# janelia-flyem/transfer_em

Hardware: AMD Instinct MI355X
Metric: CycleGAN train steps/sec on 132^3 x1 uint8 volumes (per-GPU batch of 1 volume; aggregate over GPUs) (higher is better)
Workload: dtype f32

## Files before the change

transfer_em_amd/csrc/wino.hip:

```cpp
#include "tem_common.h"
#include "wino_common.h"
#include <cmath>
#include <cstdio>
#include <cstdlib>

namespace wino {

#ifdef TEM_DEBUG_KNOBS
#define KDBG(x) (x)
#else
#define KDBG(x) 0
#endif


struct Ep32 {
  float slope;
  const float *gate; int32_t gN, gD, gH, gW; float gate_slope;
  const uint8_t *keep_mask;
  int32_t doz, doy, dox, dD, dH, dW;
  int32_t gbytes, mbytes;
};

struct Dev {
  const float *in0, *in1;
  int32_t i0N, i0D, i0H, i0W, i1N, i1D, i1H, i1W;
  int32_t C0;
  int32_t N, D, H, W;
  const float *u;
  float *out0, *out1;
  int32_t o0N, o0D, o0H, o0W, o1N, o1D, o1H, o1W;
  int32_t CO0;
  int32_t OD, OH, OW;
  int32_t P;
  int32_t BY, BX, nby, nbx, zsegs, zper, NTZ;
  int32_t E, PLC, subb, slotb;
  int32_t ndma;
  int32_t span0, span1;
  uint32_t magicBX, magicE;
  int32_t dbg;
  int32_t obytes;
  unsigned long long *stamps;
  Ep32 ep;
};

template <int CI, int CO, int NI, int EP, int EE>
__global__ __launch_bounds__(512) void wino_conv_k(Dev p) {
  constexpr int NH = CI / 8, VB = 32;
  constexpr int NB = (CO + 15) / 16;
  constexpr bool STREAM = CI == 32;
  constexpr bool PAIR = CI == 8 && CO == 8;
  constexpr int NKZ = PAIR ? 4 : 3;
  constexpr int UCH = 2 * NB * 16 * 128;
  extern __shared__ __attribute__((aligned(16))) float lds[];
  char *const ring = reinterpret_cast<char *>(lds);
  const int tid = threadIdx.x, lane = tid & 63;
  const int wave = __builtin_amdgcn_readfirstlane(tid >> 6);
  const int m = lane & 15, q = lane >> 4;
  const int grp = PAIR ? wave : (NB == 1 ? wave >> 1 : wave >> 2);
  const int nb = NB == 1 ? 0 : (wave >> 1) & 1;
  const int zb = PAIR ? (q >> 1) : (wave & 1);
  const int co = PAIR ? 4 * (q & 1) : nb * 16 + 4 * q;
  float *const uld = reinterpret_cast<float *>(ring + 4 * p.slotb);

  int seg = (int)xcd_contiguous_block(blockIdx.x, gridDim.x);
  const int zseg = seg % p.zsegs; seg /= p.zsegs;
  const int bx = seg % p.nbx; seg /= p.nbx;
  const int by = seg % p.nby;
  const int n = seg / p.nby;
  const int tz0 = zseg * p.zper, tz1 = min(p.NTZ, tz0 + p.zper), nsteps = tz1 - tz0;
  const int oy0 = by * 2 * p.BY, ox0 = bx * 2 * p.BX;
  const int ntile = p.BY * p.BX;

  const bool two_in = p.in1 != p.in0;
  const float *const in0n = p.in0 + (size_t)n * p.i0N, *const in1n = p.in1 + (size_t)n * p.i1N;
  int voff0[NI], voff1[NI];
  {
    const int iy0 = oy0 - p.P, ix0 = ox0 - p.P;
#pragma unroll
    for (int i = 0; i < NI; ++i) {
      const int sp = (wave + 8 * i) * 64 + lane;
      const bool ex = sp < p.PLC;
      const int spc = ex ? sp : 0;
      const int cpos = spc & 1, ve = spc >> 1;
      const int ro = ve / EE, e = ve - ro * EE;
      const int o = ro & 1, yr = ro >> 1;
      const int c = (cpos ^ swz(e, yr)) * 4;
      const int iy = iy0 + yr, ix = ix0 + 2 * e + o;
      const bool ok = ex && (unsigned)iy < (unsigned)p.H && (unsigned)ix < (unsigned)p.W;
      voff0[i] = ok ? (iy * p.i0H + ix * p.i0W + c) * 4 : (int)0x80000000;
      voff1[i] = ok ? (iy * p.i1H + ix * p.i1W + c) * 4 : (int)0x80000000;
      asm volatile("" : "+v"(voff0[i]), "+v"(voff1[i]));
    }
  }
  auto dma_plane = [&](int iz, int slot) {
    const bool zok = (unsigned)iz < (unsigned)p.D;
    const int izc = zok ? iz : 0;
#pragma unroll
    for (int h = 0; h < NH; ++h) {
      char *const dst = ring + slot * p.slotb + h * p.subb;
      if (!two_in || 8 * h < p.C0)
        dma_subimage<NI, !STREAM>(in0n + izc * p.i0D + 8 * h, zok ? p.span0 - 32 * h : 0, voff0, dst, wave, p.ndma);
      else
        dma_subimage<NI, !STREAM>(in1n + izc * p.i1D + (8 * h - p.C0), zok ? p.span1 - 4 * (8 * h - p.C0) : 0, voff1, dst, wave, p.ndma);
    }
  };

  const int izb0 = 2 * tz0 - p.P;
  if (nsteps > 0) {
#pragma unroll
    for (int k = 0; k < 4; ++k) dma_plane(izb0 + k, k);
  }
  auto dma_u = [&](int chunk, int buf) {
    const __amdgpu_buffer_rsrc_t r = __builtin_amdgcn_make_buffer_rsrc((void *)(p.u + (size_t)chunk * UCH), 0, UCH * 4, 0x00020000);
#pragma unroll
    for (int i = 0; i < UCH * 4 / 1024 / 8; ++i) {
      const int j = wave + 8 * i;
      __builtin_amdgcn_raw_ptr_buffer_load_lds(r, (__attribute__((address_space(3))) void *)((char *)uld + buf * (UCH * 4) + j * 1024), 16,
                                               (j * 64 + lane) * 16, 0, 0, 0);
    }
  };
  if (STREAM) {
    dma_u(0, 0);
  } else {
    constexpr int UF4 = NKZ * NH * NB * 16 * 64 * 2 / 4;
    static_assert(UF4 % 512 == 0, "whole 1 KB wave transfers");
    const __amdgpu_buffer_rsrc_t ur = __builtin_amdgcn_make_buffer_rsrc((void *)p.u, 0, UF4 * 16, 0x00020000);
#pragma unroll
    for (int i = 0; i < UF4 / 512; ++i) {
      const int j = wave + 8 * i;
      __builtin_amdgcn_raw_ptr_buffer_load_lds(ur, (__attribute__((address_space(3))) void *)((char *)uld + j * 1024), 16,
                                               (j * 64 + lane) * 16, 0, 0, 0);
    }
  }
  asm volatile("s_waitcnt vmcnt(0)" ::: "memory");
  __syncthreads();

  constexpr int rowb = EE * VB;
  const Ep32 &ep = p.ep;
  float *const out0n = p.out0 + (size_t)n * p.o0N, *const out1n = EP == 2 ? p.out1 + (size_t)n * p.o1N : nullptr;
  const float *const gaten = EP >= 1 ? ep.gate + (size_t)n * ep.gN : nullptr;
  const bool in0c = EP != 2 || co < p.CO0;
  float *const obase = EP == 2 ? (in0c ? out0n : out1n) : out0n;
  const int oco = in0c ? co : co - p.CO0;
  const int oD = in0c ? p.o0D : p.o1D, oH = in0c ? p.o0H : p.o1H, oW = in0c ? p.o0W : p.o1W;
  const __amdgpu_buffer_rsrc_t grs = __builtin_amdgcn_make_buffer_rsrc((void *)gaten, 0, EP >= 1 ? ep.gbytes : 0, 0x00020000);
  const __amdgpu_buffer_rsrc_t mrs = __builtin_amdgcn_make_buffer_rsrc((void *)ep.keep_mask, 0, EP == 2 ? ep.mbytes : 0, 0x00020000);
  const int mpv = EP == 2 ? p.CO0 >> 3 : 0;
  const int kshift = co & 4;
  int gso[4], mso[4], oso[4];
#pragma unroll
  for (int o4 = 0; o4 < 4; ++o4) {
    gso[o4] = EP >= 1 ? ((o4 >> 1) * ep.gH + (o4 & 1) * ep.gW) * 4 : 0;
    mso[o4] = EP == 2 ? ((o4 >> 1) * ep.dW + (o4 & 1)) * mpv : 0;
    oso[o4] = ((o4 >> 1) * p.o0H + (o4 & 1) * p.o0W) * 4;
  }
  const __amdgpu_buffer_rsrc_t ors = __builtin_amdgcn_make_buffer_rsrc((void *)out0n, 0, EP != 2 ? p.obytes : 0, 0x00020000);

  const int tA = min(grp * 16 + m, ntile - 1);
  const int tyA = (int)fdiv((uint32_t)tA, (uint32_t)p.BX, p.magicBX), txA = tA - tyA * p.BX;
  const int a0 = (4 * tyA * EE + txA) * VB + (q & 1) * 8;
  int cs[2][2];
#pragma unroll
  for (int a = 0; a < 2; ++a)
#pragma unroll
    for (int b = 0; b < 2; ++b) cs[a][b] = ((q >> 1) ^ swz(txA + a, 2 * (tyA + b))) * 16;

#ifdef TEM_DEBUG_KNOBS
  unsigned long long t_last = p.stamps ? clock64() : 0, t_sum[8] = {0, 0, 0, 0, 0, 0, 0, 0};
#define STAMP(i) do { if (p.stamps) { unsigned long long t_now = clock64(); t_sum[i] += t_now - t_last; t_last = t_now; } } while (0)
#else
#define STAMP(i) do { } while (0)
#endif
  f32x4 acc[16];
  f32x4 gv[4];
  uint32_t kb[4];
  uint32_t tyx, tok4 = 0;
  {
    const int t = grp * 16 + m;
    const int ty = (int)fdiv((uint32_t)t, (uint32_t)p.BX, p.magicBX), tx = t - ty * p.BX;
    const int oy = oy0 + 2 * ty, ox = ox0 + 2 * tx;
    const bool tok = co < CO && t < ntile;
#pragma unroll
    for (int o4 = 0; o4 < 4; ++o4) tok4 |= ((tok && oy + (o4 >> 1) < p.OH && ox + (o4 & 1) < p.OW) ? 1u : 0u) << o4;
    tyx = ((uint32_t)oy << 16) | (uint32_t)ox;
  }
  auto tile_geom = [&](int oz, int &o0, int &go, int &mb, uint32_t &okm) {
    uint32_t yx = tyx;
    asm volatile("" : "+v"(yx));
    const int oy = (int)(yx >> 16), ox = (int)(yx & 0xffffu);
    okm = oz < p.OD ? tok4 : 0u;
    o0 = oz * oD + oy * oH + ox * oW + oco;
    go = EP >= 1 ? (oz * ep.gD + oy * ep.gH + ox * ep.gW + co) * 4 : 0;
    mb = EP == 2 ? (int)(((((uint32_t)n * ep.dD + (oz + ep.doz)) * ep.dH + (oy + ep.doy)) * ep.dW + (ox + ep.dox)) * (uint32_t)mpv) + (co >> 3) : 0;
  };
  auto fetch_ep = [&](int oz) {
    int o0, go, mb;
    uint32_t okm;
    tile_geom(oz, o0, go, mb, okm);
    if (!in0c) okm = 0;
#pragma unroll
    for (int o4 = 0; o4 < 4; ++o4) {
      const bool okf = (okm >> o4) & 1u;
      int goff = okf ? go : (int)0x80000000;
      asm volatile("" : "+v"(goff));
      const u32x4 g4 = __builtin_amdgcn_raw_buffer_load_b128(grs, goff, gso[o4], 0);
      gv[o4] = f32x4{__uint_as_float(g4.x), __uint_as_float(g4.y), __uint_as_float(g4.z), __uint_as_float(g4.w)};
      if (EP == 2) {
        int moff = okf ? mb : (int)0x80000000;
        asm volatile("" : "+v"(moff));
        kb[o4] = (uint32_t)__builtin_amdgcn_raw_buffer_load_b8(mrs, moff, mso[o4], 0) >> kshift;
      }
    }
  };
  auto finish = [&](int oz) {
    f32x4 yx[4][2], yy[2][2];
#pragma unroll
    for (int a = 0; a < 4; ++a) at4(acc[a * 4 + 0], acc[a * 4 + 1], acc[a * 4 + 2], acc[a * 4 + 3], yx[a][0], yx[a][1]);
#pragma unroll
    for (int b = 0; b < 2; ++b) at4(yx[0][b], yx[1][b], yx[2][b], yx[3][b], yy[0][b], yy[1][b]);
    int o0, go, mb;
    uint32_t okm;
    tile_geom(oz, o0, go, mb, okm);
#pragma unroll
    for (int o4 = 0; o4 < 4; ++o4) {
      const bool ok = (okm >> o4) & 1u;
      f32x4 val = yy[o4 >> 1][o4 & 1];
#pragma unroll
      for (int r = 0; r < 4; ++r) {
        if (EP == 0) val[r] = fmaxf(val[r], ep.slope * val[r]);
        if (EP >= 1 && in0c) {
          val[r] = gv[o4][r] > 0.f ? val[r] : ep.gate_slope * val[r];
          if (EP == 2) val[r] = ((kb[o4] >> r) & 1u) ? 2.f * val[r] : 0.f;
        }
      }
      if (EP == 2 || STREAM) {
        if (ok) *reinterpret_cast<f32x4 *>(obase + o0 + (o4 >> 1) * oH + (o4 & 1) * oW) = val;
      } else {
        int so = ok ? o0 * 4 + oso[o4] : (int)0x80000000;
        asm volatile("" : "+v"(so));
        __builtin_amdgcn_raw_buffer_store_b128(u32x4{__float_as_uint(val[0]), __float_as_uint(val[1]), __float_as_uint(val[2]), __float_as_uint(val[3])},
                                               ors, so, 0, 0);
      }
    }
  };

  for (int step = 0; step < nsteps; ++step) {
    const int tz = tz0 + step, oz = 2 * tz + zb, izb = 2 * tz - p.P;
    const bool more = step + 1 < nsteps;
    const int sA = (step & 1) ? 2 : 0;
    STAMP(0);
    if (EP >= 1) fetch_ep(oz);

#pragma unroll
    for (int i = 0; i < 16; ++i) acc[i] = f32x4{0.f, 0.f, 0.f, 0.f};
#pragma unroll
    for (int kz = 0; kz < NKZ; ++kz) {
      const int pl = PAIR ? kz : zb + kz;
      const char *plane = ring + ((pl < 2 ? sA : 2 - sA) + (pl & 1)) * p.slotb + a0;
#pragma unroll
      for (int h = 0; h < NH; ++h) {
        f32x2 v[4][4];
#pragma unroll
        for (int dy = 0; dy < 4; ++dy)
#pragma unroll
          for (int dx = 0; dx < 4; ++dx)
            v[dy][dx] = *reinterpret_cast<const f32x2 *>(plane + h * p.subb + (2 * dy + (dx & 1)) * rowb + (dx >> 1) * VB + cs[dx >> 1][dy >> 1]);
        if (kz == 1 && h == NH - 1) {
          __syncthreads();
          if (more && !(KDBG(p.dbg & 4))) { dma_plane(izb + 4, sA); dma_plane(izb + 5, sA + 1); }
        }
#pragma unroll
        for (int a = 0; a < 4; ++a) bt4(v[a][0], v[a][1], v[a][2], v[a][3]);
#pragma unroll
        for (int b = 0; b < 4; ++b) bt4(v[0][b], v[1][b], v[2][b], v[3][b]);
        if (STREAM && !(h & 1)) {
          const int c = kz * 2 + (h >> 1);
          if (c > 0) __syncthreads();
          if (c < 5) dma_u(c + 1, (c + 1) & 1);
          else if (more) dma_u(0, 0);
        }
        const float *uh = STREAM ? uld + ((kz * 2 + (h >> 1)) & 1) * UCH + (((h & 1) * NB + nb) * 16) * 128 + lane * 2
                                 : uld + (((kz * NH + h) * NB + nb) * 16) * 128 + lane * 2;
        f32x2 uf[16];
#pragma unroll
        for (int pt = 0; pt < 16; ++pt) uf[pt] = *reinterpret_cast<const f32x2 *>(uh + pt * 128);
#pragma unroll
        for (int pt = 0; pt < 16; ++pt) acc[pt] = __builtin_amdgcn_mfma_f32_16x16x4f32(uf[pt].x, v[pt >> 2][pt & 3].x, acc[pt], 0, 0, 0);
#pragma unroll
        for (int pt = 0; pt < 16; ++pt) acc[pt] = __builtin_amdgcn_mfma_f32_16x16x4f32(uf[pt].y, v[pt >> 2][pt & 3].y, acc[pt], 0, 0, 0);
      }
    }
    STAMP(1);

    finish(oz);
    STAMP(3);
    asm volatile("s_waitcnt vmcnt(0)" ::: "memory");
    __syncthreads();
  }
  static_assert(!PAIR || EP <= 1, "8 -> 8: forward and gated input-gradient only");

#ifdef TEM_DEBUG_KNOBS
  if (p.stamps && lane == 0) {
    for (int i = 0; i < 8; ++i) p.stamps[((size_t)blockIdx.x * 8 + wave) * 8 + i] = t_sum[i];
  }
#endif
#undef STAMP
}

__global__ __launch_bounds__(256) void wino_weights_k(const float *theta, float *u, const tem_wino_layer *layers) {
  const tem_wino_layer L = layers[blockIdx.x];
  const int nb = blockIdx.z, NB = (L.co + 15) / 16;
  const int co = nb * 16 + (threadIdx.x & 15), ci = (threadIdx.x >> 4) + 16 * blockIdx.y;
  if (ci >= L.ci || nb >= NB) return;
  const int NH = L.ci / 8;
  const bool pair = L.ci == 8 && L.co == 8;
  const int h = ci >> 3, q = (ci & 7) >> 1, j = ci & 1;
  if (pair) {
    if (nb) return;
    const int c16 = threadIdx.x & 15, s_ = c16 >> 3, c8 = c16 & 7;
    auto g4p = [](float a, float b, float c, float (&o)[4]) {
      o[0] = a; o[1] = 0.5f * (a + b + c); o[2] = 0.5f * (a - b + c); o[3] = c;
    };
    for (int pl = 0; pl < 4; ++pl) {
      const int kz = pl - s_;
      float gy[4][4];
      if (kz >= 0 && kz <= 2) {
        float g[3][3], gx[3][4];
        for (int t9 = 0; t9 < 9; ++t9) {
          const int t = kz * 9 + t9;
          g[t9 / 3][t9 % 3] = L.flip ? theta[L.src_off + ((int64_t)(26 - t) * 8 + c8) * 8 + ci] : theta[L.src_off + ((int64_t)t * 8 + ci) * 8 + c8];
        }
        for (int a = 0; a < 3; ++a) g4p(g[a][0], g[a][1], g[a][2], gx[a]);
        for (int x = 0; x < 4; ++x) {
          float o[4];
          g4p(gx[0][x], gx[1][x], gx[2][x], o);
          for (int y = 0; y < 4; ++y) gy[y][x] = o[y];
        }
      } else {
        for (int y = 0; y < 4; ++y) for (int x = 0; x < 4; ++x) gy[y][x] = 0.f;
      }
      float *d = u + L.dst_off + ((int64_t)(pl * 16) * 64 + (q * 16 + c16)) * 2 + j;
      for (int pt = 0; pt < 16; ++pt) d[pt * 128] = gy[pt >> 2][pt & 3];
    }
    return;
  }
  auto g4 = [](float a, float b, float c, float (&o)[4]) {
    o[0] = a; o[1] = 0.5f * (a + b + c); o[2] = 0.5f * (a - b + c); o[3] = c;
  };
#pragma unroll
  for (int kz = 0; kz < 3; ++kz) {
    float g[3][3];
#pragma unroll
    for (int t9 = 0; t9 < 9; ++t9) {
      const int t = kz * 9 + t9;
      float w = 0.f;
      if (co < L.co) w = L.flip ? theta[L.src_off + ((int64_t)(26 - t) * L.co + co) * L.ci + ci]
                                : theta[L.src_off + ((int64_t)t * L.ci + ci) * L.co + co];
      g[t9 / 3][t9 % 3] = w;
    }
    float gx[3][4], gy[4][4];
#pragma unroll
    for (int a = 0; a < 3; ++a) g4(g[a][0], g[a][1], g[a][2], gx[a]);
#pragma unroll
    for (int x = 0; x < 4; ++x) {
      float o[4];
      g4(gx[0][x], gx[1][x], gx[2][x], o);
#pragma unroll
      for (int y = 0; y < 4; ++y) gy[y][x] = o[y];
    }
    float *d = u + L.dst_off + ((int64_t)(((kz * NH + h) * NB + nb) * 16) * 64 + (q * 16 + (co & 15))) * 2 + j;
#pragma unroll
    for (int pt = 0; pt < 16; ++pt) d[pt * 128] = gy[pt >> 2][pt & 3];
  }
}

constexpr int LDS_MAX = 160 * 1024;
static thread_local char *g_name = nullptr;
static thread_local int g_name_len = 0;

template <int CI, int CO, int NI>
int plan(Dev &p, double *cost, size_t *lds_bytes, int EE) {
  constexpr int NH = CI / 8, NB = (CO + 15) / 16;
  constexpr bool PAIR = CI == 8 && CO == 8;
  const size_t ubytes = CI == 32 ? (size_t)2 * (2 * NB * 16 * 128) * 4
                                 : (size_t)(PAIR ? 4 : 3) * NH * NB * 16 * 64 * 2 * 4;
  const int TY = (p.OH + 1) / 2, TX = (p.OW + 1) / 2;
  double best = 1e300;
  static const int knob_cus = tem_env_int("TEM_WINO_CUS", 256), knob_cuw = tem_env_int("TEM_WINO_CUW", 400);
  for (int by = 1; by <= TY && by <= 64; ++by)
    for (int bx = 1; bx <= TX && bx <= 64; ++bx) {
      const int nt = by * bx;
      if (nt > (PAIR ? 128 : 64 / NB)) continue;
      if (bx + 1 > EE) continue;
      const int E = EE, plv = (2 * by + 2) * 2 * E;
      const int subb = (plv * 32 + 1023) & ~1023, slotb = NH * subb;
      const size_t bytes = (size_t)4 * slotb + ubytes;
      const int ndma = subb / 1024;
      if (bytes > (size_t)LDS_MAX || ndma > 8 * NI) continue;
      const int nby = (TY + by - 1) / by, nbx = (TX + bx - 1) / bx;
      const int cols = p.N * nby * nbx;
      const int wraps = (16 % bx) ? 1 : 0;
      const double step = 2.0 * (PAIR ? 4 : 3) * NH * 32 * 45.0 * (1.0 + 0.03 * wraps) + 3500.0 + (CI == 32 ? 3000.0 : 0.0);
      const double pro = 6000.0 + (4.0 * slotb + ubytes) / 10.0;
      for (int zs = 1; zs <= p.NTZ; ++zs) {
        const int zper = (p.NTZ + zs - 1) / zs, zsegs = (p.NTZ + zper - 1) / zper;
        if (zsegs != zs) continue;
        const double t = std::ceil(cols * zsegs / (double)knob_cus) * (pro + zper * step) +
                         knob_cuw / 100.0 * (cols * zsegs / 256.0) * (pro + zper * step);
        if (t < best) {
          best = t; p.BY = by; p.BX = bx; p.nby = nby; p.nbx = nbx; p.zsegs = zsegs; p.zper = zper;
          p.E = E; p.PLC = plv * 2; p.subb = subb; p.slotb = slotb; p.ndma = ndma; *lds_bytes = (bytes + 15) & ~(size_t)15;
        }
      }
    }
  *cost = best;
  return best < 1e300 ? TEM_OK : TEM_EUNSUPPORTED;
}

template <int CI, int CO, int NI>
int plan_memo(Dev &p, double *cost, size_t *lds_bytes, int EE) {
  struct R { int rc, BY, BX, nby, nbx, zsegs, zper, E, PLC, subb, slotb, ndma; size_t lds; double cost; };
  static tem_plan_cache<5, R> cache;
  const std::array<int, 5> key{p.N, p.OH, p.OW, p.NTZ, EE};
  R r;
  if (!cache.get(key, r)) {
    r.lds = 0; r.cost = 1e300;
    r.rc = plan<CI, CO, NI>(p, &r.cost, &r.lds, EE);
    r.BY = p.BY; r.BX = p.BX; r.nby = p.nby; r.nbx = p.nbx; r.zsegs = p.zsegs; r.zper = p.zper; r.E = p.E; r.PLC = p.PLC;
    r.subb = p.subb; r.slotb = p.slotb; r.ndma = p.ndma;
    cache.put(key, r);
  } else {
    p.BY = r.BY; p.BX = r.BX; p.nby = r.nby; p.nbx = r.nbx; p.zsegs = r.zsegs; p.zper = r.zper; p.E = r.E; p.PLC = r.PLC;
    p.subb = r.subb; p.slotb = r.slotb; p.ndma = r.ndma;
  }
  *cost = r.cost; *lds_bytes = r.lds;
  return r.rc;
}

template <int CI, int CO, int NI, int EP, int EE>
static int launch(const Dev &p, size_t lds_bytes, hipStream_t st) {
  const int nblocks = p.N * p.nby * p.nbx * p.zsegs;
  auto kern = wino_conv_k<CI, CO, NI, EP, EE>;
  static bool attr_set = false;
  if (!attr_set) {
    hipError_t e = hipFuncSetAttribute((const void *)kern, hipFuncAttributeMaxDynamicSharedMemorySize, LDS_MAX);
    if (e != hipSuccess) return (int)e;
    attr_set = true;
  }
  hipLaunchKernelGGL(kern, dim3(nblocks), dim3(512), lds_bytes, st, p);
  TEM_CHECK_LAUNCH();
  return TEM_OK;
}

template <int CI, int CO, int NI, int EP>
int run_best(Dev p, hipStream_t st, bool dry) {
  static int force = -1;
  if (force < 0) force = tem_env_int("TEM_WINO_EE", 0);
  const int pitches[2] = {9, 17};
  Dev best = p;
  double cbest = 1e300;
  size_t lds_bytes = 0;
  for (int i = 0; i < 2; ++i) {
    if (force && pitches[i] != force) continue;
    Dev q = p;
    double c = 1e300;
    size_t l = 0;
    if (plan_memo<CI, CO, NI>(q, &c, &l, pitches[i]) == TEM_OK && c < cbest) { best = q; cbest = c; lds_bytes = l; }
  }
  if (cbest >= 1e300) return TEM_EUNSUPPORTED;
  p = best;
  p.magicBX = magic_for(p.BX); p.magicE = magic_for(p.E);
  if (dry) {
    if (g_name) snprintf(g_name, g_name_len, "wino_conv_k<%d, %d, %d, %d, %d>", CI, CO, NI, EP, p.E);
    return TEM_OK;
  }
  const int nblocks = p.N * p.nby * p.nbx * p.zsegs;
  if (KDBG(p.dbg & 8))
    fprintf(stderr, "wino<%d,%d,%d> O=%dx%dx%d: BY=%d BX=%d nby=%d nbx=%d zsegs=%d zper=%d blocks=%d lds=%zu\n", CI, CO, EP,
            p.OD, p.OH, p.OW, p.BY, p.BX, p.nby, p.nbx, p.zsegs, p.zper, nblocks, lds_bytes);
  return p.E == 9 ? launch<CI, CO, NI, EP, 9>(p, lds_bytes, st) : launch<CI, CO, NI, EP, 17>(p, lds_bytes, st);
}

int dispatch(const tem_conv_args *a, hipStream_t st, bool dry) {
  const tem_view &i0 = a->in0, &o0 = a->out0;
  const bool cube = a->kd == 3 && a->kh == 3 && a->kw == 3 && a->sd == 1 && a->sh == 1 && a->sw == 1 && a->pd == a->ph &&
                    a->ph == a->pw;
  if (!cube || a->w_layout != TEM_W_WINOGRAD || a->pd < 0) return TEM_EUNSUPPORTED;
  if (!fits32(i0) || !fits32(o0)) return TEM_EUNSUPPORTED;
  Dev p{};
  p.in0 = i0.ptr; p.i0N = (int)i0.sN; p.i0D = (int)i0.sD; p.i0H = (int)i0.sH; p.i0W = (int)i0.sW; p.C0 = i0.C;
  p.in1 = i0.ptr; p.i1N = p.i0N; p.i1D = p.i0D; p.i1H = p.i0H; p.i1W = p.i0W;
  int CI = i0.C;
  auto aligned = [](const tem_view &v) {
    return ((uintptr_t)v.ptr & 15) == 0 && v.sW % 4 == 0 && v.sH % 4 == 0 && v.sD % 4 == 0 && v.sN % 4 == 0 && v.C % 4 == 0;
  };
  if (!aligned(i0)) return TEM_EUNSUPPORTED;
  if (a->in1.ptr) {
    const tem_view &i1 = a->in1;
    if (i1.N != i0.N || i1.D != i0.D || i1.H != i0.H || i1.W != i0.W) return TEM_ESHAPE;
    if (!fits32(i1) || !aligned(i1)) return TEM_EUNSUPPORTED;
    p.in1 = i1.ptr; p.i1N = (int)i1.sN; p.i1D = (int)i1.sD; p.i1H = (int)i1.sH; p.i1W = (int)i1.sW;
    CI += i1.C;
    if (i0.C % 8) return TEM_EUNSUPPORTED;
  }
  p.N = i0.N; p.D = i0.D; p.H = i0.H; p.W = i0.W;
  p.span0 = (int)(((int64_t)(i0.H - 1) * p.i0H + (int64_t)(i0.W - 1) * p.i0W + i0.C) * 4);
  p.span1 = a->in1.ptr ? (int)(((int64_t)(i0.H - 1) * p.i1H + (int64_t)(i0.W - 1) * p.i1W + a->in1.C) * 4) : p.span0;
  p.u = a->w;
  p.out0 = o0.ptr; p.o0N = (int)o0.sN; p.o0D = (int)o0.sD; p.o0H = (int)o0.sH; p.o0W = (int)o0.sW; p.CO0 = o0.C;
  {
    const int64_t ospan = (int64_t)(o0.D - 1) * o0.sD + (int64_t)(o0.H - 1) * o0.sH + (int64_t)(o0.W - 1) * o0.sW + o0.C;
    if (ospan >= ((int64_t)1 << 29)) return TEM_EUNSUPPORTED;
    p.obytes = (int)(ospan * 4);
  }
  int CO = o0.C;
  if (a->out1.ptr) {
    const tem_view &o1 = a->out1;
    if (o1.N != o0.N || o1.D != o0.D || o1.H != o0.H || o1.W != o0.W) return TEM_ESHAPE;
    if (!fits32(o1)) return TEM_EUNSUPPORTED;
    p.out1 = o1.ptr; p.o1N = (int)o1.sN; p.o1D = (int)o1.sD; p.o1H = (int)o1.sH; p.o1W = (int)o1.sW;
    CO += o1.C;
  }
  if (o0.N != i0.N) return TEM_ESHAPE;
  if (o0.D != i0.D + 2 * a->pd - 2 || o0.H != i0.H + 2 * a->ph - 2 || o0.W != i0.W + 2 * a->pw - 2) return TEM_ESHAPE;
  p.OD = o0.D; p.OH = o0.H; p.OW = o0.W;
  p.NTZ = (p.OD + 1) / 2;
  p.P = a->pd;
  {
    static int dbg = -1;
    if (dbg < 0) dbg = tem_env_int("TEM_DEBUG_FLAGS", 0);
    p.dbg = dbg;
    static unsigned long long stamp_ptr = ~0ull;
    if (stamp_ptr == ~0ull) stamp_ptr = tem_env_hex("TEM_WINO_STAMP_BUF");
    p.stamps = (unsigned long long *)stamp_ptr;
  }
  const tem_epilogue &e = a->ep;
  Ep32 &q = p.ep;
  if (e.bias || e.add.ptr) return TEM_EUNSUPPORTED;
  q.slope = e.slope; q.gate_slope = e.gate_slope;
  if (!(e.slope >= 0.f && e.slope <= 1.f)) return TEM_EUNSUPPORTED;
  int EP = 0;
  if (e.gate.ptr) {
    const tem_view &g = e.gate;
    if (g.N != o0.N || g.D != o0.D || g.H != o0.H || g.W != o0.W || g.C < o0.C) return TEM_ESHAPE;
    if (!fits32(g) || e.slope != 1.f) return TEM_EUNSUPPORTED;
    q.gate = g.ptr; q.gN = (int)g.sN; q.gD = (int)g.sD; q.gH = (int)g.sH; q.gW = (int)g.sW;
    const int64_t gspan = (int64_t)(g.D - 1) * g.sD + (int64_t)(g.H - 1) * g.sH + (int64_t)(g.W - 1) * g.sW + g.C;
    if (gspan >= ((int64_t)1 << 29)) return TEM_EUNSUPPORTED;
    q.gbytes = (int)(gspan * 4);
    EP = 1;
  }
  if (e.dropout || a->out1.ptr) {
    if (!(e.dropout && e.keep_mask && e.keep_mode == 2 && a->out1.ptr && EP == 1)) return TEM_EUNSUPPORTED;
    q.keep_mask = e.keep_mask;
    q.doz = e.drop_org[0]; q.doy = e.drop_org[1]; q.dox = e.drop_org[2];
    q.dD = e.drop_dims[0] ? e.drop_dims[0] : o0.D; q.dH = e.drop_dims[0] ? e.drop_dims[1] : o0.H;
    q.dW = e.drop_dims[0] ? e.drop_dims[2] : o0.W;
    if ((int64_t)o0.N * q.dD * q.dH * q.dW * o0.C >= ((int64_t)1 << 32)) return TEM_EUNSUPPORTED;
    if (o0.C % 8) return TEM_EUNSUPPORTED;
    q.mbytes = (int)(((int64_t)o0.N * q.dD * q.dH * q.dW * o0.C + 7) / 8);
    EP = 2;
  }
#define WINO_CASE(ci, co, ni, epi) if (CI == ci && CO == co && EP == epi) return run_best<ci, co, ni, epi>(p, st, dry);
  WINO_CASE(16, 16, 2, 0) WINO_CASE(16, 16, 2, 1) WINO_CASE(16, 16, 2, 2)
  WINO_CASE(8, 8, 3, 0) WINO_CASE(8, 8, 3, 1)
  WINO_CASE(8, 16, 2, 0) WINO_CASE(8, 16, 2, 1)
  WINO_CASE(16, 8, 2, 0) WINO_CASE(16, 8, 2, 1)
  WINO_CASE(16, 32, 2, 0) WINO_CASE(16, 32, 2, 1)
  WINO_CASE(32, 32, 2, 0) WINO_CASE(32, 32, 2, 1) WINO_CASE(32, 32, 2, 2)
  WINO_CASE(32, 16, 2, 0) WINO_CASE(32, 16, 2, 1)
#undef WINO_CASE
  return TEM_EUNSUPPORTED;
}

}

int tem_conv_wino_try(const tem_conv_args *a, hipStream_t st, bool dry) { return wino::dispatch(a, st, dry); }

int tem_conv_wino_describe(const tem_conv_args *a, char *buf, int len) {
  wino::g_name = buf; wino::g_name_len = len;
  int rc = wino::dispatch(a, nullptr, true);
  wino::g_name = nullptr;
  return rc;
}

extern "C" int tem_winograd_weights(const float *theta, float *u, const tem_wino_layer *layers_dev, int32_t nlayers,
                                    tem_stream_t stream) {
  TEM_CLEAR_ERR();
  if (!theta || !u || !layers_dev || nlayers <= 0) return TEM_EINVAL;
  hipLaunchKernelGGL(wino::wino_weights_k, dim3(nlayers, 2, 2), dim3(256), 0, (hipStream_t)stream, theta, u, layers_dev);
  TEM_CHECK_LAUNCH();
  return TEM_OK;
}
```

Before: 122.3.

## Split 32-input-channel Winograd convs into two 16-channel K-half launches

```diff
diff --git a/transfer_em_amd/csrc/wino.hip b/transfer_em_amd/csrc/wino.hip
--- a/transfer_em_amd/csrc/wino.hip
+++ b/transfer_em_amd/csrc/wino.hip
@@ -37,6 +37,7 @@
   int32_t ndma;
   int32_t span0, span1;
   uint32_t magicBX, magicE;
+  int32_t ukz;
   int32_t dbg;
   int32_t obytes;
   unsigned long long *stamps;
@@ -48,6 +49,10 @@
   constexpr int NH = CI / 8, VB = 32;
   constexpr int NB = (CO + 15) / 16;
   constexpr bool STREAM = CI == 32;
+  constexpr int EPF = EP & 3;
+  constexpr bool RAW = (EP & 4) != 0, ADD = (EP & 8) != 0;
+  constexpr bool ACT = EPF == 0 && !RAW, GATE = EPF >= 1 && !RAW, KEEP = EPF == 2 && !RAW;
+  static_assert(!(RAW && ADD) && (!(RAW || ADD) || CI == 16) && (!RAW || EPF != 1), "split-K halves: 16-channel kernels");
   constexpr bool PAIR = CI == 8 && CO == 8;
   constexpr int NKZ = PAIR ? 4 : 3;
   constexpr int UCH = 2 * NB * 16 * 128;
@@ -122,14 +127,15 @@
   if (STREAM) {
     dma_u(0, 0);
   } else {
-    constexpr int UF4 = NKZ * NH * NB * 16 * 64 * 2 / 4;
+    constexpr int UF4 = NKZ * NH * NB * 16 * 64 * 2 / 4, KZF4 = UF4 / NKZ;
     static_assert(UF4 % 512 == 0, "whole 1 KB wave transfers");
-    const __amdgpu_buffer_rsrc_t ur = __builtin_amdgcn_make_buffer_rsrc((void *)p.u, 0, UF4 * 16, 0x00020000);
+    const int gap = p.ukz * 4 - KZF4 * 16;
+    const __amdgpu_buffer_rsrc_t ur = __builtin_amdgcn_make_buffer_rsrc((void *)p.u, 0, UF4 * 16 + (NKZ - 1) * gap, 0x00020000);
 #pragma unroll
     for (int i = 0; i < UF4 / 512; ++i) {
-      const int j = wave + 8 * i;
+      const int j = wave + 8 * i, s = j * 64 + lane;
       __builtin_amdgcn_raw_ptr_buffer_load_lds(ur, (__attribute__((address_space(3))) void *)((char *)uld + j * 1024), 16,
-                                               (j * 64 + lane) * 16, 0, 0, 0);
+                                               s * 16 + (s / KZF4) * gap, 0, 0, 0);
     }
   }
   asm volatile("s_waitcnt vmcnt(0)" ::: "memory");
@@ -137,24 +143,24 @@
 
   constexpr int rowb = EE * VB;
   const Ep32 &ep = p.ep;
-  float *const out0n = p.out0 + (size_t)n * p.o0N, *const out1n = EP == 2 ? p.out1 + (size_t)n * p.o1N : nullptr;
-  const float *const gaten = EP >= 1 ? ep.gate + (size_t)n * ep.gN : nullptr;
-  const bool in0c = EP != 2 || co < p.CO0;
-  float *const obase = EP == 2 ? (in0c ? out0n : out1n) : out0n;
+  float *const out0n = p.out0 + (size_t)n * p.o0N, *const out1n = EPF == 2 ? p.out1 + (size_t)n * p.o1N : nullptr;
+  const float *const gaten = GATE ? ep.gate + (size_t)n * ep.gN : nullptr;
+  const bool in0c = EPF != 2 || co < p.CO0;
+  float *const obase = EPF == 2 ? (in0c ? out0n : out1n) : out0n;
   const int oco = in0c ? co : co - p.CO0;
   const int oD = in0c ? p.o0D : p.o1D, oH = in0c ? p.o0H : p.o1H, oW = in0c ? p.o0W : p.o1W;
-  const __amdgpu_buffer_rsrc_t grs = __builtin_amdgcn_make_buffer_rsrc((void *)gaten, 0, EP >= 1 ? ep.gbytes : 0, 0x00020000);
-  const __amdgpu_buffer_rsrc_t mrs = __builtin_amdgcn_make_buffer_rsrc((void *)ep.keep_mask, 0, EP == 2 ? ep.mbytes : 0, 0x00020000);
-  const int mpv = EP == 2 ? p.CO0 >> 3 : 0;
+  const __amdgpu_buffer_rsrc_t grs = __builtin_amdgcn_make_buffer_rsrc((void *)gaten, 0, GATE ? ep.gbytes : 0, 0x00020000);
+  const __amdgpu_buffer_rsrc_t mrs = __builtin_amdgcn_make_buffer_rsrc((void *)ep.keep_mask, 0, KEEP ? ep.mbytes : 0, 0x00020000);
+  const int mpv = KEEP ? p.CO0 >> 3 : 0;
   const int kshift = co & 4;
   int gso[4], mso[4], oso[4];
 #pragma unroll
   for (int o4 = 0; o4 < 4; ++o4) {
-    gso[o4] = EP >= 1 ? ((o4 >> 1) * ep.gH + (o4 & 1) * ep.gW) * 4 : 0;
-    mso[o4] = EP == 2 ? ((o4 >> 1) * ep.dW + (o4 & 1)) * mpv : 0;
+    gso[o4] = GATE ? ((o4 >> 1) * ep.gH + (o4 & 1) * ep.gW) * 4 : 0;
+    mso[o4] = KEEP ? ((o4 >> 1) * ep.dW + (o4 & 1)) * mpv : 0;
     oso[o4] = ((o4 >> 1) * p.o0H + (o4 & 1) * p.o0W) * 4;
   }
-  const __amdgpu_buffer_rsrc_t ors = __builtin_amdgcn_make_buffer_rsrc((void *)out0n, 0, EP != 2 ? p.obytes : 0, 0x00020000);
+  const __amdgpu_buffer_rsrc_t ors = __builtin_amdgcn_make_buffer_rsrc((void *)out0n, 0, EPF != 2 ? p.obytes : 0, 0x00020000);
 
   const int tA = min(grp * 16 + m, ntile - 1);
   const int tyA = (int)fdiv((uint32_t)tA, (uint32_t)p.BX, p.magicBX), txA = tA - tyA * p.BX;
@@ -174,6 +180,7 @@
   f32x4 acc[16];
   f32x4 gv[4];
   uint32_t kb[4];
+  f32x4 pv[4];
   uint32_t tyx, tok4 = 0;
   {
     const int t = grp * 16 + m;
@@ -190,13 +197,28 @@
     const int oy = (int)(yx >> 16), ox = (int)(yx & 0xffffu);
     okm = oz < p.OD ? tok4 : 0u;
     o0 = oz * oD + oy * oH + ox * oW + oco;
-    go = EP >= 1 ? (oz * ep.gD + oy * ep.gH + ox * ep.gW + co) * 4 : 0;
-    mb = EP == 2 ? (int)(((((uint32_t)n * ep.dD + (oz + ep.doz)) * ep.dH + (oy + ep.doy)) * ep.dW + (ox + ep.dox)) * (uint32_t)mpv) + (co >> 3) : 0;
+    go = GATE ? (oz * ep.gD + oy * ep.gH + ox * ep.gW + co) * 4 : 0;
+    mb = KEEP ? (int)(((((uint32_t)n * ep.dD + (oz + ep.doz)) * ep.dH + (oy + ep.doy)) * ep.dW + (ox + ep.dox)) * (uint32_t)mpv) + (co >> 3) : 0;
   };
   auto fetch_ep = [&](int oz) {
     int o0, go, mb;
     uint32_t okm;
     tile_geom(oz, o0, go, mb, okm);
+    if (ADD) {
+#pragma unroll
+      for (int o4 = 0; o4 < 4; ++o4) {
+        const bool okp = (okm >> o4) & 1u;
+        if (EPF == 2) {
+          pv[o4] = okp ? *reinterpret_cast<const f32x4 *>(obase + o0 + (o4 >> 1) * oH + (o4 & 1) * oW) : f32x4{0.f, 0.f, 0.f, 0.f};
+        } else {
+          int so = okp ? o0 * 4 + oso[o4] : (int)0x80000000;
+          asm volatile("" : "+v"(so));
+          const u32x4 v4 = __builtin_amdgcn_raw_buffer_load_b128(ors, so, 0, 0);
+          pv[o4] = f32x4{__uint_as_float(v4.x), __uint_as_float(v4.y), __uint_as_float(v4.z), __uint_as_float(v4.w)};
+        }
+      }
+    }
+    if (!GATE) return;
     if (!in0c) okm = 0;
 #pragma unroll
     for (int o4 = 0; o4 < 4; ++o4) {
@@ -205,7 +227,7 @@
       asm volatile("" : "+v"(goff));
       const u32x4 g4 = __builtin_amdgcn_raw_buffer_load_b128(grs, goff, gso[o4], 0);
       gv[o4] = f32x4{__uint_as_float(g4.x), __uint_as_float(g4.y), __uint_as_float(g4.z), __uint_as_float(g4.w)};
-      if (EP == 2) {
+      if (KEEP) {
         int moff = okf ? mb : (int)0x80000000;
         asm volatile("" : "+v"(moff));
         kb[o4] = (uint32_t)__builtin_amdgcn_raw_buffer_load_b8(mrs, moff, mso[o4], 0) >> kshift;
@@ -227,13 +249,14 @@
       f32x4 val = yy[o4 >> 1][o4 & 1];
 #pragma unroll
       for (int r = 0; r < 4; ++r) {
-        if (EP == 0) val[r] = fmaxf(val[r], ep.slope * val[r]);
-        if (EP >= 1 && in0c) {
+        if (ADD) val[r] = pv[o4][r] + val[r];
+        if (ACT) val[r] = fmaxf(val[r], ep.slope * val[r]);
+        if (GATE && in0c) {
           val[r] = gv[o4][r] > 0.f ? val[r] : ep.gate_slope * val[r];
-          if (EP == 2) val[r] = ((kb[o4] >> r) & 1u) ? 2.f * val[r] : 0.f;
+          if (KEEP) val[r] = ((kb[o4] >> r) & 1u) ? 2.f * val[r] : 0.f;
         }
       }
-      if (EP == 2 || STREAM) {
+      if (EPF == 2 || STREAM) {
         if (ok) *reinterpret_cast<f32x4 *>(obase + o0 + (o4 >> 1) * oH + (o4 & 1) * oW) = val;
       } else {
         int so = ok ? o0 * 4 + oso[o4] : (int)0x80000000;
@@ -249,7 +272,7 @@
     const bool more = step + 1 < nsteps;
     const int sA = (step & 1) ? 2 : 0;
     STAMP(0);
-    if (EP >= 1) fetch_ep(oz);
+    if (GATE || ADD) fetch_ep(oz);
 
 #pragma unroll
     for (int i = 0; i < 16; ++i) acc[i] = f32x4{0.f, 0.f, 0.f, 0.f};
@@ -386,7 +409,7 @@
                                  : (size_t)(PAIR ? 4 : 3) * NH * NB * 16 * 64 * 2 * 4;
   const int TY = (p.OH + 1) / 2, TX = (p.OW + 1) / 2;
   double best = 1e300;
-  static const int knob_cus = tem_env_int("TEM_WINO_CUS", 256), knob_cuw = tem_env_int("TEM_WINO_CUW", 400);
+  static const int knob_cus = tem_env_int("TEM_WINO_CUS", 256), knob_cuw = tem_env_int("TEM_WINO_CUW", 100);
   for (int by = 1; by <= TY && by <= 64; ++by)
     for (int bx = 1; bx <= TX && bx <= 64; ++bx) {
       const int nt = by * bx;
@@ -452,33 +475,90 @@
   return TEM_OK;
 }
 
-template <int CI, int CO, int NI, int EP>
-int run_best(Dev p, hipStream_t st, bool dry) {
+template <int CI, int CO, int NI>
+double choose(Dev &p, size_t *lds_bytes) {
   static int force = -1;
   if (force < 0) force = tem_env_int("TEM_WINO_EE", 0);
   const int pitches[2] = {9, 17};
   Dev best = p;
   double cbest = 1e300;
-  size_t lds_bytes = 0;
   for (int i = 0; i < 2; ++i) {
     if (force && pitches[i] != force) continue;
     Dev q = p;
     double c = 1e300;
     size_t l = 0;
-    if (plan_memo<CI, CO, NI>(q, &c, &l, pitches[i]) == TEM_OK && c < cbest) { best = q; cbest = c; lds_bytes = l; }
-  }
-  if (cbest >= 1e300) return TEM_EUNSUPPORTED;
+    if (plan_memo<CI, CO, NI>(q, &c, &l, pitches[i]) == TEM_OK && c < cbest) { best = q; cbest = c; *lds_bytes = l; }
+  }
   p = best;
   p.magicBX = magic_for(p.BX); p.magicE = magic_for(p.E);
+  p.ukz = (CI / 8) * ((CO + 15) / 16) * 16 * 128;
+  return cbest;
+}
+
+template <int CI, int CO, int NI, int EP>
+static int launch_plan(const Dev &p, size_t lds_bytes, hipStream_t st) {
+  if (KDBG(p.dbg & 8))
+    fprintf(stderr, "wino<%d,%d,%d> O=%dx%dx%d: BY=%d BX=%d nby=%d nbx=%d zsegs=%d zper=%d blocks=%d lds=%zu\n", CI, CO, EP,
+            p.OD, p.OH, p.OW, p.BY, p.BX, p.nby, p.nbx, p.zsegs, p.zper, p.N * p.nby * p.nbx * p.zsegs, lds_bytes);
+  return p.E == 9 ? launch<CI, CO, NI, EP, 9>(p, lds_bytes, st) : launch<CI, CO, NI, EP, 17>(p, lds_bytes, st);
+}
+
+template <int CI, int CO, int NI, int EP>
+int run_best(Dev p, hipStream_t st, bool dry) {
+  size_t lds_bytes = 0;
+  if (choose<CI, CO, NI>(p, &lds_bytes) >= 1e300) return TEM_EUNSUPPORTED;
   if (dry) {
     if (g_name) snprintf(g_name, g_name_len, "wino_conv_k<%d, %d, %d, %d, %d>", CI, CO, NI, EP, p.E);
     return TEM_OK;
   }
-  const int nblocks = p.N * p.nby * p.nbx * p.zsegs;
-  if (KDBG(p.dbg & 8))
-    fprintf(stderr, "wino<%d,%d,%d> O=%dx%dx%d: BY=%d BX=%d nby=%d nbx=%d zsegs=%d zper=%d blocks=%d lds=%zu\n", CI, CO, EP,
-            p.OD, p.OH, p.OW, p.BY, p.BX, p.nby, p.nbx, p.zsegs, p.zper, nblocks, lds_bytes);
-  return p.E == 9 ? launch<CI, CO, NI, EP, 9>(p, lds_bytes, st) : launch<CI, CO, NI, EP, 17>(p, lds_bytes, st);
+  return launch_plan<CI, CO, NI, EP>(p, lds_bytes, st);
+}
+
+template <int CO, int EP>
+int run_32(Dev p, hipStream_t st, bool dry) {
+  static int force = -2;
+  if (force == -2) force = tem_env_int("TEM_WINO_SPLITK", -1);
+  constexpr int NB = (CO + 15) / 16;
+  Dev s = p, h = p;
+  size_t ls = 0, lh = 0;
+  const double cs = force == 1 ? 1e300 : choose<32, CO, 2>(s, &ls);
+  double ch = 1e300;
+  const bool two_in = p.in1 != p.in0;
+  if (force != 0 && (!two_in || p.C0 == 16)) {
+    ch = choose<16, CO, 2>(h, &lh);
+    static const int knob_cuw = tem_env_int("TEM_WINO_CUW", 100);
+    const double rmw = 2.0 * 4.0 * CO * (double)p.N * p.OD * p.OH * p.OW;
+    if (ch < 1e300) ch = 2.0 * ch + (1.0 + knob_cuw / 100.0) * rmw / (10.0 * 256.0);
+  }
+  if (cs >= 1e300 && ch >= 1e300) return TEM_EUNSUPPORTED;
+  if (cs <= ch) {
+    if (dry) {
+      if (g_name) snprintf(g_name, g_name_len, "wino_conv_k<32, %d, 2, %d, %d>", CO, EP, s.E);
+      return TEM_OK;
+    }
+    return launch_plan<32, CO, 2, EP>(s, ls, st);
+  }
+  constexpr int EP0 = (EP == 2 ? 2 : 0) | 4, EP1 = EP | 8;
+  if (dry) {
+    if (g_name) snprintf(g_name, g_name_len, "wino_conv_k<16, %d, 2, %d+%d, %d>", CO, EP0, EP1, h.E);
+    return TEM_OK;
+  }
+  h.C0 = 16;
+  h.ukz = 2 * (2 * NB * 16 * 128);
+  Dev h1 = h;
+  h.in1 = h.in0; h.i1N = h.i0N; h.i1D = h.i0D; h.i1H = h.i0H; h.i1W = h.i0W;
+  if (two_in) {
+    h1.in0 = p.in1; h1.i0N = p.i1N; h1.i0D = p.i1D; h1.i0H = p.i1H; h1.i0W = p.i1W;
+  } else {
+    h1.in0 = p.in0 + 16;
+  }
+  h1.in1 = h1.in0; h1.i1N = h1.i0N; h1.i1D = h1.i0D; h1.i1H = h1.i0H; h1.i1W = h1.i0W;
+  h1.u = p.u + 2 * NB * 16 * 128;
+  h.span0 = h.span1 = (int)(((int64_t)(p.H - 1) * h.i0H + (int64_t)(p.W - 1) * h.i0W + 16) * 4);
+  h1.span0 = h1.span1 = (int)(((int64_t)(p.H - 1) * h1.i0H + (int64_t)(p.W - 1) * h1.i0W + 16) * 4);
+  const int rc = launch_plan<16, CO, 2, EP0>(h, lh, st);
+  if (rc != TEM_OK) return rc;
+  return launch_plan<16, CO, 2, EP1>(h1, lh, st);
 }
 
 int dispatch(const tem_conv_args *a, hipStream_t st, bool dry) {
@@ -567,9 +647,11 @@
   WINO_CASE(8, 16, 2, 0) WINO_CASE(8, 16, 2, 1)
   WINO_CASE(16, 8, 2, 0) WINO_CASE(16, 8, 2, 1)
   WINO_CASE(16, 32, 2, 0) WINO_CASE(16, 32, 2, 1)
-  WINO_CASE(32, 32, 2, 0) WINO_CASE(32, 32, 2, 1) WINO_CASE(32, 32, 2, 2)
-  WINO_CASE(32, 16, 2, 0) WINO_CASE(32, 16, 2, 1)
 #undef WINO_CASE
+#define WINO_CASE32(co, epi) if (CI == 32 && CO == co && EP == epi) return run_32<co, epi>(p, st, dry);
+  WINO_CASE32(32, 0) WINO_CASE32(32, 1) WINO_CASE32(32, 2)
+  WINO_CASE32(16, 0) WINO_CASE32(16, 1)
+#undef WINO_CASE32
   return TEM_EUNSUPPORTED;
 }
 
```

Result: faster. 124.1 (median of 6 runs) (+1.5%).
